# RustAudio/lewton

Measured on NVIDIA H100. Metric: Msamples/s IMDCT+window+OLA, 2048-pt long blocks, higher is better.
Workload: dtype f32

## Files before the change

lewton_b200/csrc/host_objects.cuh:

```cuda
#pragma once

struct DevBuf {
    void *p = nullptr;
    size_t cap = 0;
};

struct Staging {
    void *h = nullptr;
    size_t cap = 0;
    cudaEvent_t ev = nullptr;
    bool pending = false;
};

struct ArenaSet {
    DevBuf coeffs, dense, pcm, kinds, ys, vqoff, vqrec;
    cudaEvent_t done = nullptr;
};
constexpr int kHostSets = 2;

struct CachedTables {
    DevTables dt;
    std::vector<float> a, b, c, w;
    std::vector<uint32_t> br;
    std::vector<void *> allocs;
// ... 38 lines not shown
    lwb_ctx *ctx = nullptr;
    DevSetup host;
    DevSetup *d_setup = nullptr;
    std::vector<void *> allocs;
    uint8_t channels = 0, bs0 = 0, bs1 = 0;
    uint32_t n_modes = 0;
    uint32_t n_mappings = 0;
    std::vector<DevMapping> mappings;
    std::vector<uint8_t> floor_types;
    std::vector<DevFloor0> floor0;
    mutable bool streams_opened = false;
    bool floor0_described(uint32_t fi) const { return fi < floor0.size() && floor0[fi].order != 0; }
    unsigned out_channels() const { return host.n_out ? host.n_out : channels; }
};

struct RowCopy { const void *src; void *dst; uint64_t bytes; };
constexpr int kRowCopyThreads = 256;
struct ChainShape { unsigned warps; size_t smem; int n1max, wpc, np; };

struct Step {
    int kernel;
    const void *desc;
    size_t n;
    const float *pack;
};

struct StepArgs {
    void *pcm = nullptr;
    int out_format = LWB_OUT_F32_PLANAR;
    const float *w_short = nullptr;
    int ls = 0;
// ... 29 lines not shown
    lwb_batch_io io;
    bool captured = false;
    uint64_t gen = 0;
    FrontStages front;
    DevBuf pro, desc;
    StepArgs args;
    std::vector<Step> steps;
};

struct lwb_stream {
    lwb_ctx *ctx = nullptr;
    const lwb_setup *setup = nullptr;
    float *d_state = nullptr;
    bool has = false;
    uint32_t plen = 0;
    uint64_t busy_epoch = 0;
    uint64_t skip_left = 0;
    uint64_t limit_left = ~0ull;
};

static void capture(lwb_plan *plan, uint64_t gen, const FrontStages &front, const StepArgs &args, std::vector<Step> steps)
{
    plan->captured = true;
    plan->gen = gen;
    plan->front = front;
    for (size_t i = 0; i < plan->n_chains && front.n; i++)
        if (!plan->chains[i].stream->setup->floor0.empty()) plan->front.floor0 = true;
    plan->args = args;
    plan->steps = std::move(steps);
}


static inline void set_stream_state(lwb_stream *s, bool has, uint32_t plen)
{
    if (s->has != has || s->plen != plen) {
        s->has = has;
        s->plen = plen;
        s->ctx->state_gen++;
    }
}

static int fail(lwb_ctx *ctx, int code, const char *what, cudaError_t e = cudaSuccess)
{
    if (ctx) {
        ctx->err = what;
        if (e != cudaSuccess) {
            ctx->err += ": ";
            ctx->err += cudaGetErrorString(e);
        }
    }
    return code;
}
// ... 190 lines not shown
```

lewton_b200/csrc/kernel_long.cuh:

```cuda
#pragma once
#include <stdint.h>

#include "lwb_common.h"

#if defined(__CUDACC__)
#include <cuda_fp16.h>
#include <cuda_runtime.h>

#include <type_traits>
#define LWB_HD __host__ __device__ __forceinline__
#else
#define LWB_HD inline
#endif

namespace lwb {

constexpr int kLongBs = 11;
constexpr int kLongN = 2048;
constexpr int kLongN2 = 1024;

struct alignas(16) LongRun {
    const float *in;
    void *out;
    float *state;
    uint32_t in_stride;
    uint32_t n_packets;
    uint8_t has_prev;
    uint8_t write_state;
    uint8_t dummy;
    uint8_t first_short;
    uint8_t last_short;
    uint8_t pad[3];
    float *state_out;
};
static_assert(sizeof(LongRun) == 48, "LongRun is copied by TMA in 16-byte units");

struct V { float x, y; };

#if defined(__CUDA_ARCH__)
__device__ __forceinline__ V vadd(V a, V b) { return V{__fadd_rn(a.x, b.x), __fadd_rn(a.y, b.y)}; }
__device__ __forceinline__ V vsub(V a, V b) { return V{__fsub_rn(a.x, b.x), __fsub_rn(a.y, b.y)}; }
__device__ __forceinline__ V vmul(V a, V b) { return V{__fmul_rn(a.x, b.x), __fmul_rn(a.y, b.y)}; }
__device__ __forceinline__ V vadd_p(V a, V b) { return V{__fadd_rn(a.x, b.x), __fadd_rn(a.y, b.y)}; }
__device__ __forceinline__ V vsub_p(V a, V b) { return V{__fsub_rn(a.x, b.x), __fsub_rn(a.y, b.y)}; }
__device__ __forceinline__ V vnsub_p(V a, V b) { return V{__fsub_rn(-a.x, b.x), __fsub_rn(-a.y, b.y)}; }
#else
inline V vadd(V a, V b) { return V{a.x + b.x, a.y + b.y}; }
inline V vsub(V a, V b) { return V{a.x - b.x, a.y - b.y}; }
inline V vmul(V a, V b) { return V{a.x * b.x, a.y * b.y}; }
inline V vadd_p(V a, V b) { return vadd(a, b); }
// ... 348 lines not shown
__device__ __forceinline__ void mbar_wait(uint32_t bar, uint32_t parity)
{
    asm volatile(
        "{\n\t.reg .pred p;\n\t"
        "WAIT_%=:\n\t"
        "mbarrier.try_wait.parity.shared::cta.b64 p, [%0], %1, %2;\n\t"
        "@p bra DONE_%=;\n\t"
        "bra WAIT_%=;\n\t"
        "DONE_%=:\n\t}" ::"r"(bar), "r"(parity), "r"(200000u) : "memory");
}
__device__ __forceinline__ void tma_load_1d(uint32_t dst, const void *src, uint32_t bytes, uint32_t bar)
{
    asm volatile("cp.async.bulk.shared::cluster.global.mbarrier::complete_tx::bytes [%0], [%1], %2, [%3];"
                 ::"r"(dst), "l"(src), "r"(bytes), "r"(bar) : "memory");
}
__device__ __forceinline__ void fence_proxy_async()
{
    asm volatile("fence.proxy.async.shared::cta;" ::: "memory");
}
__device__ __forceinline__ void sts_eo(uint32_t addr, float e, float o)
{
    asm volatile("st.shared.f32 [%0], %1;\n\tst.shared.f32 [%0+2048], %2;" ::"r"(addr), "f"(e), "f"(o) : "memory");
}
__device__ __forceinline__ void lds_eo(uint32_t addr, float &e, float &o)
{
    asm volatile("ld.shared.f32 %0, [%2];\n\tld.shared.f32 %1, [%2+2048];" : "=f"(e), "=f"(o) : "r"(addr) : "memory");
}

}
#include "kernel_deal.cuh"
// ... 77 lines not shown
    case kSampleI16: return f(SampleType<int16_t>());
    case kSampleF16: return f(SampleType<__half>());
    default: return f(SampleType<float>());
    }
}

template <int FORMAT>
__device__ __forceinline__ void store_sample(void *pcm, uint64_t off, uint64_t stride, unsigned channels, unsigned ch,
                                             uint64_t i, float v)
{
    constexpr OutFormat F = out_format_of(FORMAT);
    using T = sample_t<F.kind>;
    static_cast<T *>(pcm)[off + (F.planar ? (uint64_t)ch * stride + i : i * channels + ch)] = d_sample(v, static_cast<T *>(nullptr));
}

template <int Wd, int TOP, bool FIRST, typename OutT>
__device__ __forceinline__ void out_block(const TwMix &tw, int hl, const V O[8], const V E[8], V pe[8], uint32_t flags,
                                          OutT *out, const float *s_state)
{
#pragma unroll
    for (int j = 0; j < 8; j++) {
        const int rw = Wd * rev3(j);
        const bool nat = (j & 1);
        const V b0 = tw(P_B0 + j), b1 = tw(P_B1 + j);
        const V wlo = tw(P_WLO + j), whi = tw(P_WHI + j);
        V plo = pe[j], phi = pe[j];
        bool emit = !(flags & 4u);
        if (FIRST) {
            emit = emit && (flags & 1u);
            if (flags & 1u) {
                const float *s_lo = s_state + hl, *s_hi = s_state + Wd - 1 - hl;
                const float ax = nat ? s_lo[rw] : s_hi[rw], ay = nat ? s_hi[rw] : s_lo[rw];
                const float bx = nat ? s_hi[TOP - rw] : s_lo[TOP - rw];
                const float by = nat ? s_lo[TOP - rw] : s_hi[TOP - rw];
                plo = V{ax, ay};
                phi = V{bx, by};
            }
        }
        V lo, hi, pev;
        step8_ola(b0, b1, wlo, whi, O[j], E[j], plo, phi, lo, hi, pev);
        pe[j] = pev;
        if (emit) {
            OutT *o_lo = out + hl, *o_hi = out + Wd - 1 - hl;
            if (nat) {
                st_pcm(o_lo + rw, lo.x); st_pcm(o_hi + rw, lo.y);
                st_pcm(o_hi + TOP - rw, hi.x); st_pcm(o_lo + TOP - rw, hi.y);
            } else {
                st_pcm(o_hi + rw, lo.x); st_pcm(o_lo + rw, lo.y);
                st_pcm(o_lo + TOP - rw, hi.x); st_pcm(o_hi + TOP - rw, hi.y);
            }
        }
    }
}

template <int NB, bool FIRST, typename OutT, typename RC>
__device__ __forceinline__ void out_stage(const TwMix &tw, int lane, const V O[NB][8], const V E[NB][8], V pe[NB][8],
                                          const RC cur[NB], OutT *out[NB], const float *s_state)
{
#pragma unroll
    for (int b = 0; b < NB; b++)
        out_block<64, kLongN2 - 64, FIRST>(tw, lane, O[b], E[b], pe[b], cur[b].flags, out[b], s_state + b * kLongN2);
}

__device__ __forceinline__ float lds_f32(uint32_t addr)
{
    float v;
    asm volatile("ld.shared.f32 %0, [%1];" : "=f"(v) : "r"(addr) : "memory");
    return v;
}

template <int NB, typename OutT, typename RC = RunCur, bool EXPORT = false, int LS = 0>
__device__ __forceinline__ void out_first_short(const TwMix &tw, int lane, const V O[NB][8], const V E[NB][8], V pe[NB][8],
                                                const RC cur[NB], OutT *out[NB], const float *s_state,
                                                const float *__restrict__ w, int ls_arg, uint32_t w_s = 0)
{
    const int ls = LS ? LS : ls_arg;
// ... 71 lines not shown
        }
    }
    __syncwarp();
#pragma unroll
    for (int b = 0; b < NB; b++) {
        const uint32_t c0 = stage_s + b * kLongTileBytes + lC0, c1 = stage_s + b * kLongTileBytes + lC1;
#pragma unroll
        for (int j = 0; j < 8; j++) {
            lds_eo(c0 ^ LWB_KC(j), E[b][j].x, O[b][j].x);
            lds_eo(c1 ^ LWB_KC(j), E[b][j].y, O[b][j].y);
        }
    }
    __syncwarp();
}

template <int Wd, int TOP>
__device__ __forceinline__ void store_right_half(float *state, int hl, const V pe[8])
{
    float *s_lo = state + hl, *s_hi = state + Wd - 1 - hl;
#pragma unroll
    for (int j = 0; j < 8; j++) {
        const int rw = Wd * rev3(j);
        const float vx = (j & 1) ? pe[j].x : pe[j].y, vy = (j & 1) ? pe[j].y : pe[j].x;
        s_lo[rw] = vx; s_hi[rw] = vy;
        s_hi[TOP - rw] = vx; s_lo[TOP - rw] = vy;
    }
}

template <int LS, typename OutT>
__device__ __forceinline__ void end_of_run(int lane, const V pe[8], uint32_t flags, uint32_t npk, OutT *out, float *state, int ls_arg)
{
    static_assert(LS % 64 == 0, "LS must be a multiple of 64");
    const int ls = LS ? LS : ls_arg;
    if (flags & 16u) {
        const bool emitted = (npk > 1 || (flags & 1u)) && !(flags & 4u);
        const bool keep = (flags & 6u) == 2u;
#pragma unroll
        for (int j = 0; j < 8; j++) {
            const int r64 = 64 * rev3(j);
#pragma unroll
            for (int h = 0; h < 2; h++) {
                const float v = ((j & 1) != 0) == (h == 0) ? pe[j].x : pe[j].y;
                const int m = r64 + (h ? 63 - lane : lane);
                if (LS ? (r64 < LS) : (m < ls)) {
                    if (emitted) st_pcm(out + m, v);
                } else if (keep && m < kLongN2 - ls) {
                    state[m - ls] = v;
                    state[kLongN2 - 1 - ls - m] = v;
                }
            }
        }
    } else if ((flags & 6u) == 2u) {
        store_right_half<64, kLongN2 - 64>(state, lane, pe);
    }
}

template <int Ring, size_t StageBytes, size_t Desc>
struct LongSmem {
    static constexpr size_t kTilesBytes = (size_t)kLongWarps * Ring * StageBytes;
    static constexpr size_t kStateBytes = (size_t)kLongWarps * StageBytes;
    static constexpr size_t kDescBytes = (size_t)kLongWarps * Desc * sizeof(LongRun);
    float *tiles, *s_state;
    V *s_pack;
    LongRun *s_desc;
    uint64_t *bars;
    unsigned char *rest;
    __device__ __forceinline__ LongSmem(unsigned char *smem_raw, int warp)
    {
// ... 69 lines not shown
    const uint32_t state_s = smem_u32(s_state), next_s = smem_u32(s_next);
    const uint32_t lA0 = laneA(lane, 0), lA1 = laneA(lane, 1);
    const uint32_t lB = laneB(lane);
    const uint32_t lC0 = laneC(lane, 0), lC1 = laneC(lane, 1);
    uint32_t phase_bits = 0;
    uint32_t slot_i = 0;

    uint32_t lc = 0;
    uint32_t nx_idx = 0;
    uint32_t nx_stage = 0;
    uint32_t nx_lc = 0, nx_npk = 0;
    uint32_t nx_state_issued = 0;
    uint32_t desc_parity = 0;
    RunCur cur[NB];
    uint32_t npk;

    auto issue_stage = [&](uint32_t stage, const auto *r, uint32_t pkt) {
        const uint32_t bar = bars_s + 8 * stage;
        mbar_expect_tx(bar, kLongStageBytes);
#pragma unroll
        for (int b = 0; b < NB; b++)
            tma_load_1d(tiles_s + stage * kLongStageBytes + b * kLongTileBytes,
                        r[b].in + (size_t)pkt * r[b].in_stride, kLongTileBytes, bar);
    };
    auto issue_state = [&](const float *const st[NB], const uint32_t has[NB]) {
        uint32_t bytes = 0;
#pragma unroll
        for (int b = 0; b < NB; b++) bytes += has[b] ? kLongTileBytes : 0;
        mbar_expect_tx(bar_state, bytes);
#pragma unroll
        for (int b = 0; b < NB; b++)
            if (has[b]) tma_load_1d(state_s + b * kLongTileBytes, st[b], kLongTileBytes, bar_state);
    };
    auto request_desc = [&]() {
        if (nx_idx < n_groups) {
            fence_proxy_async();
            mbar_expect_tx(bar_desc, NB * (uint32_t)sizeof(LongRun));
            tma_load_1d(next_s, runs + (size_t)nx_idx * NB, NB * (uint32_t)sizeof(LongRun), bar_desc);
            nx_stage = 1;
        } else {
            nx_stage = 3;
        }
    };
    auto land_desc = [&]() {
        mbar_wait(bar_desc, desc_parity);
        desc_parity ^= 1u;
        nx_stage = 2;
        nx_npk = s_next[0].n_packets;
        nx_lc = 0;
    };
    auto request_state = [&]() {
        const float *st[NB];
        uint32_t has[NB];
#pragma unroll
        for (int b = 0; b < NB; b++) { st[b] = s_next[b].state; has[b] = s_next[b].has_prev; }
        fence_proxy_async();
        issue_state(st, has);
        nx_state_issued = 1;
    };

    {
        uint32_t idx = 0;
        if (lane == 0) idx = atomicAdd(ticket, 1u);
        idx = __shfl_sync(0xffffffffu, idx, 0);
        if (idx >= n_groups) return;
#pragma unroll
        for (int b = 0; b < NB; b++) cur[b] = run_cur(runs[idx * NB + b]);
        npk = runs[idx * NB].n_packets;
        if (lane == 0) {
            fence_proxy_async();
            const float *st[NB];
            uint32_t has[NB];
#pragma unroll
            for (int b = 0; b < NB; b++) { st[b] = cur[b].state; has[b] = cur[b].flags & 1u; }
            issue_state(st, has);
            for (; lc < (uint32_t)kLongRing && lc < npk; lc++) issue_stage(lc, cur, lc);
            nx_idx = atomicAdd(ticket, 1u);
        }
    }

    for (;;) {
        V pe[NB][8];
#pragma unroll
        for (int b = 0; b < NB; b++)
#pragma unroll
            for (int j = 0; j < 8; j++) pe[b][j] = V{0.f, 0.f};
        OutT *out[NB];
#pragma unroll
        for (int b = 0; b < NB; b++) out[b] = static_cast<OutT *>(cur[b].out);

// ... 26 lines not shown
                            fence_proxy_async();
                            issue_stage(tgt, s_next, nx_lc);
                            nx_lc++;
                        }
                    }
                }
            }
            phase_c_fft<NB>(tw, O, E);
            if (p > 0) {
                out_stage<NB, false>(tw, lane, O, E, pe, cur, out, s_state);
            } else {
                mbar_wait(bar_state, (phase_bits >> 30) & 1u);
                phase_bits ^= 1u << 30;
                if (NB == 1 && (cur[0].flags & 8u))
                    out_first_short<NB, OutT>(tw, lane, O, E, pe, cur, out, s_state, w_short, ls);
                else
                    out_stage<NB, true>(tw, lane, O, E, pe, cur, out, s_state);
                __syncwarp();
            }
#pragma unroll
            for (int b = 0; b < NB; b++)
                if (p > 0 || (cur[b].flags & 1u)) out[b] += (p == 0 && (cur[b].flags & 8u)) ? kLongN2 - ls : kLongN2;
            if (lane == 0 && nx_stage == 2 && !nx_state_issued) request_state();
            slot_i = (slot_i + 1 == (uint32_t)kLongRing) ? 0 : slot_i + 1;
        }
#pragma unroll
        for (int b = 0; b < NB; b++) end_of_run<0>(lane, pe[b], cur[b].flags, npk, out[b], cur[b].state, ls);
        uint32_t st_ = 0, nlc = 0;
        if (lane == 0) {
            if (nx_stage == 0) request_desc();
            if (nx_stage == 1) land_desc();
            if (nx_stage == 2 && !nx_state_issued) request_state();
            st_ = nx_stage;
            nlc = nx_lc;
        }
        st_ = __shfl_sync(0xffffffffu, st_, 0);
        nlc = __shfl_sync(0xffffffffu, nlc, 0);
        if (st_ != 2) break;
        __syncwarp();
#pragma unroll
        for (int b = 0; b < NB; b++) cur[b] = run_cur(s_next[b]);
        npk = s_next[0].n_packets;
        __syncwarp();
        lc = nlc;
        nx_stage = 0; nx_lc = 0; nx_npk = 0; nx_state_issued = 0;
        if (lane == 0) {
            fence_proxy_async();
            for (uint32_t k = lc; k < (uint32_t)kLongRing && k < npk; k++) {
                issue_stage((slot_i + k) % kLongRing, cur, k);
                lc = k + 1;
            }
            nx_idx = atomicAdd(ticket, 1u);
        }
    }
}

// ... 138 lines not shown
```

lewton_b200/csrc/lwb_api.cu:

```cuda
#include <cuda_runtime.h>
#include <sched.h>
#include <sys/syscall.h>
#include <unistd.h>

#include <algorithm>
#include <cctype>
#include <cmath>
#include <cstdio>
#include <cstdlib>
#include <cstring>
#include <deque>
#include <new>
#include <string>
#include <vector>

#include "kernel_long.cuh"
#include "kernel_short.cuh"
#include "kernel_mid.cuh"
#include "kernels_generic.cuh"
#include "kernel_chain.cuh"
#include "kernel_prologue.cuh"
#include "kernel_floor0.cuh"
#include "lwb_common.h"
#include "pcm_copy_plan.h"
// ... 528 lines not shown
}

extern "C" void lwb_stream_destroy(lwb_stream *s)
{
    if (!s) return;
    cudaSetDevice(s->ctx->device);
    sync_all_streams(s->ctx);
    cudaFree(s->d_state);
    delete s;
}

extern "C" int lwb_stream_reset(lwb_stream *s)
{
    if (!s) return LWB_ERR_INVALID;
    set_stream_state(s, false, 0);
    return LWB_OK;
}
extern "C" int lwb_stream_set_window(lwb_stream *s, uint64_t skip, uint64_t limit)
{
    if (!s) return LWB_ERR_INVALID;
    s->skip_left = skip;
    s->limit_left = limit;
    s->ctx->windows_set = true;
    s->ctx->state_gen++;
    return LWB_OK;
}
extern "C" int lwb_stream_window(const lwb_stream *s, uint64_t *skip_left, uint64_t *limit_left)
{
    if (!s) return LWB_ERR_INVALID;
    if (skip_left) *skip_left = s->skip_left;
    if (limit_left) *limit_left = s->limit_left;
    return LWB_OK;
}
extern "C" int lwb_stream_is_empty(const lwb_stream *s) { return (!s || !s->has) ? 1 : 0; }
extern "C" uint32_t lwb_stream_state_len(const lwb_stream *s) { return (s && s->has) ? s->plen : 0; }

extern "C" int lwb_stream_clone(const lwb_stream *s, lwb_stream **out)
{
    if (!s || !out) return LWB_ERR_INVALID;
    int rc = lwb_stream_open(s->ctx, s->setup, out);
    if (rc) return rc;
    (*out)->has = s->has;
    (*out)->plen = s->plen;
    (*out)->skip_left = s->skip_left;
    (*out)->limit_left = s->limit_left;
    lwb_ctx *ctx = s->ctx;
    CU(ctx, cudaMemcpyAsync((*out)->d_state, s->d_state,
                            s->setup->channels * state_stride(s->setup) * sizeof(float),
                            cudaMemcpyDeviceToDevice, ctx->stream));
    return LWB_OK;
}

extern "C" int lwb_stream_export_state(lwb_stream *s, float *out)
{
    if (!s || !out) return LWB_ERR_INVALID;
    if (!s->has) return LWB_OK;
    lwb_ctx *ctx = s->ctx;
    CU(ctx, cudaSetDevice(ctx->device));
    CU(ctx, cudaMemcpy2DAsync(out, s->plen * sizeof(float), s->d_state, state_stride(s->setup) * sizeof(float),
                              s->plen * sizeof(float), s->setup->channels, cudaMemcpyDeviceToHost, ctx->stream));
    CU(ctx, cudaStreamSynchronize(ctx->stream));
    return LWB_OK;
}

extern "C" int lwb_stream_import_state(lwb_stream *s, const float *data, uint32_t len)
{
    if (!s || (!data && len)) return LWB_ERR_INVALID;
    if (len > state_stride(s->setup)) return LWB_ERR_BUFFER;
    lwb_ctx *ctx = s->ctx;
    CU(ctx, cudaSetDevice(ctx->device));
    if (len) {
        CU(ctx, cudaMemcpy2DAsync(s->d_state, state_stride(s->setup) * sizeof(float), data, len * sizeof(float),
                                  len * sizeof(float), s->setup->channels, cudaMemcpyHostToDevice, ctx->stream));
        CU(ctx, cudaStreamSynchronize(ctx->stream));
    }
    s->ctx->state_gen++;
    s->has = true;
    s->plen = len;
    return LWB_OK;
}

extern "C" int lwb_decoded_sample_count(const lwb_setup *su, uint8_t mode, int prev_flag, int next_flag,
                                        uint32_t *n_samples)
{
    if (!su || !n_samples) return LWB_ERR_INVALID;
    Geom g;
    int rc = geometry(su, mode, prev_flag, next_flag, &g);
    if (rc) return rc;
    *n_samples = g.rs - g.ls;
    return LWB_OK;
}

#include "path_generic.cuh"
// ... 122 lines not shown
static int queue_batch(lwb_ctx *ctx, lwb_chain *chains, size_t n_chains, const lwb_batch_io *io, lwb_plan *prepared, bool pinned_only)
{
    if (!ctx || (!chains && n_chains) || !io) return LWB_ERR_INVALID;
    BatchWalk bw;
    int rc = walk_batch(ctx, chains, n_chains, io, pinned_only, &bw);
    if (rc || n_chains == 0) return rc;
    CU(ctx, cudaSetDevice(ctx->device));
    if ((rc = place_clipped_chains(ctx, chains, n_chains, io, &bw))) return rc;
    const lwb_chain *decode = bw.clip.empty() ? chains : bw.clip.data();
    if (prepared) prepared->captured = false;
    size_t first = first_batch_path();
    for (size_t i = 0; i < n_chains && first < kChainPath; i++)
        if (chains[i].stream->setup->host.n_out) first = kChainPath;
    for (size_t k = first; k < std::size(kBatchPaths); k++) {
        bool handled = false;
        if ((rc = kBatchPaths[k](ctx, decode, n_chains, io, bw, &handled, prepared))) return rc;
        if (!handled) continue;
        if (prepared && !bw.clip.empty()) prepared->captured = false;
        for (size_t i = 0; i < n_chains; i++) set_chain_result(&chains[i], bw.walks[i]);
        commit_stream_states(chains, bw.walks);
        return LWB_OK;
    }
    return fail(ctx, LWB_ERR_INVALID, "internal: no batch path took the batch");
}

static int decode_chains_impl(lwb_ctx *ctx, lwb_chain *chains, size_t n_chains, const lwb_batch_io *io, lwb_plan *prepared,
                              uint64_t *ticket = nullptr)
{
    if (!ctx) return LWB_ERR_INVALID;
    const uint64_t issued = ctx->tickets_issued;
    int rc = queue_batch(ctx, chains, n_chains, io, prepared, ticket != nullptr);
    if (rc) return rc;
    if (!ticket) return ctx->tickets_issued != issued ? retire_tickets(ctx, ctx->tickets_issued, true) : LWB_OK;
    if (ctx->tickets_issued == issued) {
        CU(ctx, cudaSetDevice(ctx->device));
// ... 71 lines not shown
{
    size_t rows = 0;
    for (size_t i = 0; i < n; i++)
        if (slot_len(slots[i], load)) rows += slots[i].stream->setup->channels;
    if (!rows) return LWB_OK;
    Staging *st;
    int rc;
    if ((rc = acquire_staging(ctx, rows * sizeof(RowCopy), &st)) || (rc = ensure(ctx, ctx->state_rows, rows * sizeof(RowCopy)))) return rc;
    RowCopy *h = (RowCopy *)st->h;
    size_t k = 0;
    for (size_t i = 0; i < n; i++) {
        const lwb_stream *s = slots[i].stream;
        const uint32_t len = slot_len(slots[i], load);
        for (unsigned c = 0; len && c < s->setup->channels; c++) {
            float *row = s->d_state + (size_t)c * state_stride(s->setup), *b = dev + (slots[i].offset - base) + (uint64_t)c * len;
            h[k++] = load ? RowCopy{b, row, len * sizeof(float)} : RowCopy{row, b, len * sizeof(float)};
        }
    }
    if ((rc = upload_staging(ctx, st, h, ctx->state_rows.p, rows * sizeof(RowCopy), ctx->stream))) return rc;
    return run_steps(ctx, StepArgs(), std::vector<Step>(1, Step{LWB_KERNEL_ROW_COPY, ctx->state_rows.p, rows, nullptr}));
}

static int move_states(lwb_ctx *ctx, bool load, lwb_state_slot *slots_w, const lwb_state_slot *slots, size_t n, int memory, float *buf,
                       uint64_t *ticket)
{
    uint64_t lo, hi;
    int rc = check_state_slots(ctx, slots, n, memory, buf, ticket, load, &lo, &hi);
    if (rc) return rc;
    CU(ctx, cudaSetDevice(ctx->device));
    ArenaSet *set = nullptr;
    if (memory == LWB_MEM_DEVICE || hi <= lo) {
// ... 26 lines not shown
            }
        }
        if (rc) {
            cudaEventRecord(set->done, ctx->stream);
            cudaGetLastError();
            return rc;
        }
    }
    if ((rc = issue_ticket(ctx, set))) return rc;
    *ticket = ctx->tickets_issued;
    for (size_t i = 0; i < n; i++) {
        lwb_stream *s = slots[i].stream;
        if (load) {
            s->has = slots[i].has != 0;
            s->plen = slots[i].len;
        } else {
            slots_w[i].len = slot_len(slots[i], false);
            slots_w[i].has = s->has ? 1 : 0;
        }
    }
    if (load) ctx->state_gen++;
    return LWB_OK;
}

extern "C" int lwb_streams_save(lwb_ctx *ctx, lwb_state_slot *slots, size_t n, int memory, float *buf, uint64_t *ticket)
{
    return move_states(ctx, false, slots, slots, n, memory, buf, ticket);
}

extern "C" int lwb_streams_load(lwb_ctx *ctx, const lwb_state_slot *slots, size_t n, int memory, const float *buf, uint64_t *ticket)
// ... 189 lines not shown
```

lewton_b200/csrc/path_chain.cuh:

```cuda
#pragma once

static size_t chain_smem(unsigned maxc, int n1max, int np, bool vq = false)
{
    return (size_t)maxc * ((size_t)np * n1max + n1max / 2) * 4 + 8 * (LWB_MAX_POSTS + 1) * 2 * 2 + 64 +
           (vq ? (size_t)maxc * (n1max / 2) * 4 : 0);
}
static int chain_np(unsigned maxc, int n1max, int wpc, bool residue)
{
    if (residue || wpc != 1) return 1;
    int np = 4;
    while (np > 1 && chain_smem(maxc, n1max, np) > 64 * 1024) np >>= 1;
    return np;
}
static ChainShape chain_shape(unsigned maxc, int n1max, bool residue, bool vq = false)
{
    int wpc = std::max(1, std::min(8, n1max / 1024));
    while (wpc > 1 && (unsigned)wpc * maxc > 32) wpc >>= 1;
    const int np = chain_np(maxc, n1max, wpc, residue);
    return ChainShape{maxc * wpc, chain_smem(maxc, n1max, np, vq), n1max, wpc, np};
}

template <int Q>
__device__ __forceinline__ void row_copy_shifted(const uint4 *__restrict__ a, uint4 *__restrict__ d, uint64_t nv, unsigned r)
{
    for (uint64_t v = threadIdx.x; v < nv; v += blockDim.x) {
        const uint4 A = a[v], B = a[v + 1];
        const uint32_t w[8] = {A.x, A.y, A.z, A.w, B.x, B.y, B.z, B.w};
        d[v] = make_uint4(__funnelshift_r(w[Q], w[Q + 1], r), __funnelshift_r(w[Q + 1], w[Q + 2], r), __funnelshift_r(w[Q + 2], w[Q + 3], r),
                          __funnelshift_r(w[Q + 3], w[Q + 4], r));
    }
}

__global__ void __launch_bounds__(kRowCopyThreads) k_row_copy(const RowCopy *__restrict__ rc)
{
    const RowCopy c = rc[blockIdx.x];
    const char *src = static_cast<const char *>(c.src);
    char *dst = static_cast<char *>(c.dst);
    const uint64_t head = min(c.bytes, (uint64_t)((16 - (reinterpret_cast<uintptr_t>(dst) & 15)) & 15));
    const uint64_t nv = (c.bytes - head) >> 4;
    for (uint64_t i = 2 * threadIdx.x; i < head; i += 2 * blockDim.x)
        *reinterpret_cast<uint16_t *>(dst + i) = *reinterpret_cast<const uint16_t *>(src + i);
    for (uint64_t i = head + nv * 16 + 2 * threadIdx.x; i < c.bytes; i += 2 * blockDim.x)
        *reinterpret_cast<uint16_t *>(dst + i) = *reinterpret_cast<const uint16_t *>(src + i);
    uint4 *d = reinterpret_cast<uint4 *>(dst + head);
    const char *s = src + head;
    const unsigned sh = reinterpret_cast<uintptr_t>(s) & 15, r = (sh & 3) * 8;
    const uint4 *a = reinterpret_cast<const uint4 *>(s - sh);
    switch (sh >> 2) {
    case 0:
        if (!sh) {
// ... 123 lines not shown
```

lewton_b200/csrc/path_generic.cuh:

```cuda
#pragma once

struct ChainWalk {
    uint32_t done = 0;
    int status = LWB_OK;
    uint64_t n_samples = 0;
    uint64_t skip = 0;
    uint64_t written = 0;
    bool end_has = false;
    uint32_t end_plen = 0;
    bool clear_after = false;
    uint64_t coeff_end = 0;
    uint32_t full_n = 0;
    bool long_only = true;
    bool clipped() const { return skip || written != n_samples; }
};

template <typename F>
static ChainWalk walk_chain(const lwb_chain *c, F &&on_packet)
{
    const lwb_setup *su = c->stream->setup;
    ChainWalk w;
    bool has = c->stream->has;
    uint32_t plen = c->stream->plen;
    uint64_t coeff = c->coeff_offset, pos = 0;
// ... 398 lines not shown
    for (size_t i = i0; i < i1; i++) {
        const lwb_chain *c = &chains[i];
        pcm_chain_spans(planar, c->stream->setup->out_channels(), c->out_offset, c->out_stride, walks[i].written, ctx->pcm_spans);
    }
    plan_pcm_copies(ctx->pcm_spans, (uint64_t)INT32_MAX / esz, ctx->pcm_copies);
    for (const PcmCopy &cp : ctx->pcm_copies) {
        char *dst = (char *)io->pcm + cp.off * esz;
        const char *src = (const char *)stage + (cp.off - obase) * esz;
        if (cp.height == 1) CU(ctx, cudaMemcpyAsync(dst, src, cp.width * esz, cudaMemcpyDeviceToHost, st));
        else CU(ctx, cudaMemcpy2DAsync(dst, cp.pitch * esz, src, cp.pitch * esz, cp.width * esz, cp.height, cudaMemcpyDeviceToHost, st));
    }
    return LWB_OK;
}

static int run_steps(lwb_ctx *ctx, const StepArgs &a, const std::vector<Step> &steps);

struct BatchArenas {
    const float *coeffs = nullptr, *dense = nullptr;
    char *pcm = nullptr;
    FloorViews fl;
    lwb_ctx *ctx = nullptr;
    const lwb_batch_io *io = nullptr;
    ArenaSet *set = nullptr;
    bool host = false;
    unsigned C = 0;
    uint64_t c_lo = 0, o_lo = 0;
    cudaStream_t up = nullptr, down = nullptr;

    int open(lwb_ctx *ctx_, const lwb_batch_io *io_, const BatchExtent &ext, unsigned C_, bool copy_streams)
    {
// ... 412 lines not shown
```

lewton_b200/csrc/path_long.cuh:

```cuda
#pragma once

struct LongItem {
    const lwb_chain *c;
    uint32_t P;
    bool has_prev;
};

static void long_runs_of(const LongItem &it, size_t cuts, const float *coeffs, char *pcm, size_t esz, LongRun *&w)
{
    for (unsigned ch = 0; ch < it.c->stream->setup->channels; ch++, w += cuts)
        channel_run(it.c, ch, kLongN2, coeffs + it.c->coeff_offset, pcm, esz, it.P, it.has_prev, it.has_prev ? kLongN2 : 0, cuts, w);
}

static bool batch_is_uniform_long(const lwb_chain *chains, size_t n_chains, const lwb_batch_io *io, const BatchWalk &bw)
{
    if (!fused_layout(chains, n_chains, io)) return false;
    const float *pack = nullptr;
    for (size_t i = 0; i < n_chains; i++) {
        const lwb_chain *c = &chains[i];
        const lwb_stream *s = c->stream;
        const lwb_setup *su = s->setup;
        if (su->bs1 != kLongBs || !su->host.tab[1].pack) return false;
        if (pack && pack != su->host.tab[1].pack) return false;
        pack = su->host.tab[1].pack;
        if (s->has && s->plen != (uint32_t)kLongN2) return false;
        if (bw.walks[i].done != c->n_packets || !bw.walks[i].long_only) return false;
    }
    return true;
}

struct LongRuns {
    struct Chunk { size_t r0, nr; };
    std::vector<Chunk> chunks;
    Staging *st = nullptr;
    LongRun *h = nullptr, *d = nullptr;
    size_t n = 0;
    int par = 0;
    bool own = false;
};

static int long_build_runs(lwb_ctx *ctx, const lwb_chain *chains, size_t n_chains, size_t n_chunks, const float *coeffs, char *pcm,
                           size_t esz, DevBuf *own, LongRuns *lr)
{
    std::vector<LongItem> items;
    items.reserve(n_chains);
    size_t chan_chains = 0;
    for (size_t i = 0; i < n_chains; i++) {
        const lwb_chain *c = &chains[i];
        items.push_back(LongItem{c, c->n_packets, c->stream->has});
        if (c->n_packets) chan_chains += c->stream->setup->channels;
    }
    const size_t warp_slots = (size_t)ctx->sm_count * kLongWarps * kLongNB;
    size_t target_runs = warp_slots * 4;
    if (const char *e = getenv("LWB_LONG_TARGET_RUNS")) target_runs = (size_t)atol(e);
    const size_t min_run = 8;
    int rc;
    std::vector<size_t> cuts(items.size(), 1);
// ... 18 lines not shown
    lr->h = h_runs;
    std::vector<LongRun> tmp;
    std::vector<uint32_t> order;
    for (size_t k = 0; k < n_chunks; k++) {
        const size_t i0 = items.size() * k / n_chunks, i1 = items.size() * (k + 1) / n_chunks;
        LongRun *w0 = w;
        size_t chunk_runs = 0;
        for (size_t i = i0; i < i1; i++)
            if (items[i].P) chunk_runs += cuts[i] * items[i].c->stream->setup->channels;
        LongRun *gen = w;
        if (kLongNB > 1) {
            tmp.resize(chunk_runs);
            gen = tmp.data();
        }
        for (size_t i = i0; i < i1; i++)
            if (items[i].P) long_runs_of(items[i], cuts[i], coeffs, pcm, esz, gen);
        if (kLongNB == 1) {
            w = gen;
        } else {
            bool sorted = true;
            for (size_t i = 1; i < tmp.size() && sorted; i++) sorted = tmp[i].n_packets == tmp[0].n_packets;
            order.resize(tmp.size());
            for (uint32_t i = 0; i < order.size(); i++) order[i] = i;
            if (!sorted)
                std::stable_sort(order.begin(), order.end(),
                                 [&](uint32_t a, uint32_t b) { return tmp[a].n_packets < tmp[b].n_packets; });
            size_t i = 0;
            while (i < order.size()) {
                size_t j = i;
                while (j < order.size() && tmp[order[j]].n_packets == tmp[order[i]].n_packets) j++;
                for (size_t q = i; q < j; q++) *w++ = tmp[order[q]];
// ... 60 lines not shown
    StepArgs args;
    args.pcm = ar.pcm;
    args.out_format = io->out_format;
    std::vector<Step> steps;
    LongRuns lr;
    uint64_t gen = 0;
    size_t pk0 = 0;
    for (size_t k = 0; k < n_chunks; k++) {
        const size_t i0 = n_chains * k / n_chunks, i1 = n_chains * (k + 1) / n_chunks;
        const BatchExtent ke = chunk_extent(io, chains, bw, i0, i1);
        if (ke.empty()) continue;
        size_t npk = 0;
        for (size_t i = i0; i < i1; i++) npk += chains[i].n_packets;
        if ((rc = ar.upload(k, ke)) || (residue && (rc = front_stages_launch(ctx, ar, fs, pk0, npk)))) return rc;
        if (!lr.d) {
            if ((rc = long_build_runs(ctx, chains, n_chains, n_chunks, in, ar.pcm, out_format_of(io->out_format).esz, cap ? &plan->desc : nullptr, &lr)) ||
                (rc = long_upload_runs(ctx, lr, host ? ctx->copy_in : ctx->copy_out)))
                return rc;
            gen = ctx->state_gen;
        }
        steps.assign(1, Step{LWB_KERNEL_LONG, lr.d + lr.chunks[k].r0, lr.chunks[k].nr / kLongNB, pack});
        if ((rc = run_steps(ctx, args, steps)) || (rc = ar.download(k, bw, i0, i1, ke))) return rc;
        pk0 += npk;
    }
    CU(ctx, cudaEventRecord(ctx->ev_kdone[lr.par], ctx->stream));
    if (cap) capture(plan, gen, fs, args, std::move(steps));
    return ar.finish();
}
```

Before: 323,500.

## Store only half of long-block overlap state and mirror it lazily

The long-block kernel keeps only the non-redundant half of the symmetric overlap-add state when running under a captured plan. It writes half the state rows with an L2 evict_last hint and reads them back with half-size TMA loads. Other batch paths, state export and slot save rebuild the full mirrored rows through a mirror mode in the row-copy kernel. This halves state traffic per run, but adds a stream flag, generation bumps and an extra mirroring launch whenever a non-long path reads the state.

New measurement: 332,000 (median of 6 runs). +2.6%, better.

```diff
diff --git a/lewton_b200/csrc/host_objects.cuh b/lewton_b200/csrc/host_objects.cuh
--- a/lewton_b200/csrc/host_objects.cuh
+++ b/lewton_b200/csrc/host_objects.cuh
@@ -76,7 +76,7 @@
     unsigned out_channels() const { return host.n_out ? host.n_out : channels; }
 };
 
-struct RowCopy { const void *src; void *dst; uint64_t bytes; };
+struct RowCopy { const void *src; void *dst; uint64_t bytes; bool mirror = false; };
 constexpr int kRowCopyThreads = 256;
 struct ChainShape { unsigned warps; size_t smem; int n1max, wpc, np; };
 
@@ -136,6 +136,7 @@
     float *d_state = nullptr;
     bool has = false;
     uint32_t plen = 0;
+    bool half = false;
     uint64_t busy_epoch = 0;
     uint64_t skip_left = 0;
     uint64_t limit_left = ~0ull;
@@ -158,6 +159,14 @@
     if (s->has != has || s->plen != plen) {
         s->has = has;
         s->plen = plen;
+        s->ctx->state_gen++;
+    }
+}
+
+static inline void set_stream_half(lwb_stream *s, bool half)
+{
+    if (s->half != half) {
+        s->half = half;
         s->ctx->state_gen++;
     }
 }
diff --git a/lewton_b200/csrc/kernel_long.cuh b/lewton_b200/csrc/kernel_long.cuh
--- a/lewton_b200/csrc/kernel_long.cuh
+++ b/lewton_b200/csrc/kernel_long.cuh
@@ -30,10 +30,12 @@
     uint8_t dummy;
     uint8_t first_short;
     uint8_t last_short;
-    uint8_t pad[3];
+    uint8_t half;
+    uint8_t pad[2];
     float *state_out;
 };
 static_assert(sizeof(LongRun) == 48, "LongRun is copied by TMA in 16-byte units");
+constexpr uint8_t kLongHalfIn = 1, kLongHalfOut = 2;
 
 struct V { float x, y; };
 
@@ -412,6 +414,16 @@
     asm volatile("cp.async.bulk.shared::cluster.global.mbarrier::complete_tx::bytes [%0], [%1], %2, [%3];"
                  ::"r"(dst), "l"(src), "r"(bytes), "r"(bar) : "memory");
 }
+__device__ __forceinline__ uint64_t l2_evict_last_policy()
+{
+    uint64_t p;
+    asm volatile("createpolicy.fractional.L2::evict_last.b64 %0, 1.0;" : "=l"(p));
+    return p;
+}
+__device__ __forceinline__ void st_f32_policy(float *p, float v, uint64_t pol)
+{
+    asm volatile("st.global.L2::cache_hint.f32 [%0], %1, %2;" ::"l"(p), "f"(v), "l"(pol) : "memory");
+}
 __device__ __forceinline__ void fence_proxy_async()
 {
     asm volatile("fence.proxy.async.shared::cta;" ::: "memory");
@@ -519,7 +531,7 @@
     static_cast<T *>(pcm)[off + (F.planar ? (uint64_t)ch * stride + i : i * channels + ch)] = d_sample(v, static_cast<T *>(nullptr));
 }
 
-template <int Wd, int TOP, bool FIRST, typename OutT>
+template <int Wd, int TOP, bool FIRST, typename OutT, bool HALF = false>
 __device__ __forceinline__ void out_block(const TwMix &tw, int hl, const V O[8], const V E[8], V pe[8], uint32_t flags,
                                           OutT *out, const float *s_state)
 {
@@ -536,10 +548,14 @@
             if (flags & 1u) {
                 const float *s_lo = s_state + hl, *s_hi = s_state + Wd - 1 - hl;
                 const float ax = nat ? s_lo[rw] : s_hi[rw], ay = nat ? s_hi[rw] : s_lo[rw];
-                const float bx = nat ? s_hi[TOP - rw] : s_lo[TOP - rw];
-                const float by = nat ? s_lo[TOP - rw] : s_hi[TOP - rw];
                 plo = V{ax, ay};
-                phi = V{bx, by};
+                if (HALF) {
+                    phi = plo;
+                } else {
+                    const float bx = nat ? s_hi[TOP - rw] : s_lo[TOP - rw];
+                    const float by = nat ? s_lo[TOP - rw] : s_hi[TOP - rw];
+                    phi = V{bx, by};
+                }
             }
         }
         V lo, hi, pev;
@@ -558,13 +574,13 @@
     }
 }
 
-template <int NB, bool FIRST, typename OutT, typename RC>
+template <int NB, bool FIRST, bool HALF = false, typename OutT, typename RC>
 __device__ __forceinline__ void out_stage(const TwMix &tw, int lane, const V O[NB][8], const V E[NB][8], V pe[NB][8],
                                           const RC cur[NB], OutT *out[NB], const float *s_state)
 {
 #pragma unroll
     for (int b = 0; b < NB; b++)
-        out_block<64, kLongN2 - 64, FIRST>(tw, lane, O[b], E[b], pe[b], cur[b].flags, out[b], s_state + b * kLongN2);
+        out_block<64, kLongN2 - 64, FIRST, OutT, HALF>(tw, lane, O[b], E[b], pe[b], cur[b].flags, out[b], s_state + b * kLongN2);
 }
 
 __device__ __forceinline__ float lds_f32(uint32_t addr)
@@ -666,7 +682,7 @@
     __syncwarp();
 }
 
-template <int Wd, int TOP>
+template <int Wd, int TOP, bool HALF = false>
 __device__ __forceinline__ void store_right_half(float *state, int hl, const V pe[8])
 {
     float *s_lo = state + hl, *s_hi = state + Wd - 1 - hl;
@@ -674,12 +690,17 @@
     for (int j = 0; j < 8; j++) {
         const int rw = Wd * rev3(j);
         const float vx = (j & 1) ? pe[j].x : pe[j].y, vy = (j & 1) ? pe[j].y : pe[j].x;
-        s_lo[rw] = vx; s_hi[rw] = vy;
-        s_hi[TOP - rw] = vx; s_lo[TOP - rw] = vy;
-    }
-}
-
-template <int LS, typename OutT>
+        if (HALF) {
+            const uint64_t pol = l2_evict_last_policy();
+            st_f32_policy(s_lo + rw, vx, pol); st_f32_policy(s_hi + rw, vy, pol);
+        } else {
+            s_lo[rw] = vx; s_hi[rw] = vy;
+            s_hi[TOP - rw] = vx; s_lo[TOP - rw] = vy;
+        }
+    }
+}
+
+template <int LS, bool HALF = false, typename OutT>
 __device__ __forceinline__ void end_of_run(int lane, const V pe[8], uint32_t flags, uint32_t npk, OutT *out, float *state, int ls_arg)
 {
     static_assert(LS % 64 == 0, "LS must be a multiple of 64");
@@ -703,7 +724,8 @@
             }
         }
     } else if ((flags & 6u) == 2u) {
-        store_right_half<64, kLongN2 - 64>(state, lane, pe);
+        if (HALF && (flags & 128u)) store_right_half<64, kLongN2 - 64, true>(state, lane, pe);
+        else store_right_half<64, kLongN2 - 64>(state, lane, pe);
     }
 }
 
@@ -803,6 +825,11 @@
     uint32_t desc_parity = 0;
     RunCur cur[NB];
     uint32_t npk;
+    auto run_cur_l = [](const LongRun &r) {
+        RunCur c = run_cur(r);
+        if (NB == 1) c.flags |= (uint32_t)(r.half & (kLongHalfIn | kLongHalfOut)) << 6;
+        return c;
+    };
 
     auto issue_stage = [&](uint32_t stage, const auto *r, uint32_t pkt) {
         const uint32_t bar = bars_s + 8 * stage;
@@ -812,14 +839,17 @@
             tma_load_1d(tiles_s + stage * kLongStageBytes + b * kLongTileBytes,
                         r[b].in + (size_t)pkt * r[b].in_stride, kLongTileBytes, bar);
     };
-    auto issue_state = [&](const float *const st[NB], const uint32_t has[NB]) {
-        uint32_t bytes = 0;
-#pragma unroll
-        for (int b = 0; b < NB; b++) bytes += has[b] ? kLongTileBytes : 0;
+    auto issue_state = [&](const float *const st[NB], const uint32_t fl[NB]) {
+        uint32_t bytes = 0, sz[NB];
+#pragma unroll
+        for (int b = 0; b < NB; b++) {
+            sz[b] = !(fl[b] & 1u) ? 0u : (fl[b] & 64u) ? kLongTileBytes / 2 : kLongTileBytes;
+            bytes += sz[b];
+        }
         mbar_expect_tx(bar_state, bytes);
 #pragma unroll
         for (int b = 0; b < NB; b++)
-            if (has[b]) tma_load_1d(state_s + b * kLongTileBytes, st[b], kLongTileBytes, bar_state);
+            if (sz[b]) tma_load_1d(state_s + b * kLongTileBytes, st[b], sz[b], bar_state);
     };
     auto request_desc = [&]() {
         if (nx_idx < n_groups) {
@@ -840,11 +870,11 @@
     };
     auto request_state = [&]() {
         const float *st[NB];
-        uint32_t has[NB];
-#pragma unroll
-        for (int b = 0; b < NB; b++) { st[b] = s_next[b].state; has[b] = s_next[b].has_prev; }
+        uint32_t fl[NB];
+#pragma unroll
+        for (int b = 0; b < NB; b++) { st[b] = s_next[b].state; fl[b] = run_cur_l(s_next[b]).flags; }
         fence_proxy_async();
-        issue_state(st, has);
+        issue_state(st, fl);
         nx_state_issued = 1;
     };
 
@@ -854,15 +884,15 @@
         idx = __shfl_sync(0xffffffffu, idx, 0);
         if (idx >= n_groups) return;
 #pragma unroll
-        for (int b = 0; b < NB; b++) cur[b] = run_cur(runs[idx * NB + b]);
+        for (int b = 0; b < NB; b++) cur[b] = run_cur_l(runs[idx * NB + b]);
         npk = runs[idx * NB].n_packets;
         if (lane == 0) {
             fence_proxy_async();
             const float *st[NB];
-            uint32_t has[NB];
-#pragma unroll
-            for (int b = 0; b < NB; b++) { st[b] = cur[b].state; has[b] = cur[b].flags & 1u; }
-            issue_state(st, has);
+            uint32_t fl[NB];
+#pragma unroll
+            for (int b = 0; b < NB; b++) { st[b] = cur[b].state; fl[b] = cur[b].flags; }
+            issue_state(st, fl);
             for (; lc < (uint32_t)kLongRing && lc < npk; lc++) issue_stage(lc, cur, lc);
             nx_idx = atomicAdd(ticket, 1u);
         }
@@ -919,6 +949,8 @@
                 phase_bits ^= 1u << 30;
                 if (NB == 1 && (cur[0].flags & 8u))
                     out_first_short<NB, OutT>(tw, lane, O, E, pe, cur, out, s_state, w_short, ls);
+                else if (NB == 1 && (cur[0].flags & 64u))
+                    out_stage<NB, true, true>(tw, lane, O, E, pe, cur, out, s_state);
                 else
                     out_stage<NB, true>(tw, lane, O, E, pe, cur, out, s_state);
                 __syncwarp();
@@ -930,7 +962,7 @@
             slot_i = (slot_i + 1 == (uint32_t)kLongRing) ? 0 : slot_i + 1;
         }
 #pragma unroll
-        for (int b = 0; b < NB; b++) end_of_run<0>(lane, pe[b], cur[b].flags, npk, out[b], cur[b].state, ls);
+        for (int b = 0; b < NB; b++) end_of_run<0, true>(lane, pe[b], cur[b].flags, npk, out[b], cur[b].state, ls);
         uint32_t st_ = 0, nlc = 0;
         if (lane == 0) {
             if (nx_stage == 0) request_desc();
@@ -944,7 +976,7 @@
         if (st_ != 2) break;
         __syncwarp();
 #pragma unroll
-        for (int b = 0; b < NB; b++) cur[b] = run_cur(s_next[b]);
+        for (int b = 0; b < NB; b++) cur[b] = run_cur_l(s_next[b]);
         npk = s_next[0].n_packets;
         __syncwarp();
         lc = nlc;
diff --git a/lewton_b200/csrc/lwb_api.cu b/lewton_b200/csrc/lwb_api.cu
--- a/lewton_b200/csrc/lwb_api.cu
+++ b/lewton_b200/csrc/lwb_api.cu
@@ -566,6 +566,7 @@
 {
     if (!s) return LWB_ERR_INVALID;
     set_stream_state(s, false, 0);
+    set_stream_half(s, false);
     return LWB_OK;
 }
 extern "C" int lwb_stream_set_window(lwb_stream *s, uint64_t skip, uint64_t limit)
@@ -594,6 +595,7 @@
     if (rc) return rc;
     (*out)->has = s->has;
     (*out)->plen = s->plen;
+    (*out)->half = s->half;
     (*out)->skip_left = s->skip_left;
     (*out)->limit_left = s->limit_left;
     lwb_ctx *ctx = s->ctx;
@@ -612,6 +614,8 @@
     CU(ctx, cudaMemcpy2DAsync(out, s->plen * sizeof(float), s->d_state, state_stride(s->setup) * sizeof(float),
                               s->plen * sizeof(float), s->setup->channels, cudaMemcpyDeviceToHost, ctx->stream));
     CU(ctx, cudaStreamSynchronize(ctx->stream));
+    for (unsigned c = 0; s->half && c < s->setup->channels; c++)
+        for (uint32_t m = 0; m < s->plen / 2; m++) out[(size_t)c * s->plen + s->plen - 1 - m] = out[(size_t)c * s->plen + m];
     return LWB_OK;
 }
 
@@ -629,6 +633,7 @@
     s->ctx->state_gen++;
     s->has = true;
     s->plen = len;
+    s->half = false;
     return LWB_OK;
 }
 
@@ -781,11 +786,17 @@
         if (chains[i].stream->setup->host.n_out) first = kChainPath;
     for (size_t k = first; k < std::size(kBatchPaths); k++) {
         bool handled = false;
+        if (kBatchPaths[k] != try_long &&
+            (rc = materialise_halves(ctx, n_chains, [&](size_t i) { return chains[i].stream; }, [&](size_t i) { return bw.walks[i].done > 0; })))
+            return rc;
         if ((rc = kBatchPaths[k](ctx, decode, n_chains, io, bw, &handled, prepared))) return rc;
         if (!handled) continue;
         if (prepared && !bw.clip.empty()) prepared->captured = false;
         for (size_t i = 0; i < n_chains; i++) set_chain_result(&chains[i], bw.walks[i]);
         commit_stream_states(chains, bw.walks);
+        if (kBatchPaths[k] == try_long)
+            for (size_t i = 0; i < n_chains; i++)
+                if (bw.walks[i].done) set_stream_half(chains[i].stream, prepared != nullptr);
         return LWB_OK;
     }
     return fail(ctx, LWB_ERR_INVALID, "internal: no batch path took the batch");
@@ -887,7 +898,7 @@
         const uint32_t len = slot_len(slots[i], load);
         for (unsigned c = 0; len && c < s->setup->channels; c++) {
             float *row = s->d_state + (size_t)c * state_stride(s->setup), *b = dev + (slots[i].offset - base) + (uint64_t)c * len;
-            h[k++] = load ? RowCopy{b, row, len * sizeof(float)} : RowCopy{row, b, len * sizeof(float)};
+            h[k++] = load ? RowCopy{b, row, len * sizeof(float)} : RowCopy{row, b, len * sizeof(float), s->half};
         }
     }
     if ((rc = upload_staging(ctx, st, h, ctx->state_rows.p, rows * sizeof(RowCopy), ctx->stream))) return rc;
@@ -944,6 +955,7 @@
         if (load) {
             s->has = slots[i].has != 0;
             s->plen = slots[i].len;
+            s->half = false;
         } else {
             slots_w[i].len = slot_len(slots[i], false);
             slots_w[i].has = s->has ? 1 : 0;
diff --git a/lewton_b200/csrc/path_chain.cuh b/lewton_b200/csrc/path_chain.cuh
--- a/lewton_b200/csrc/path_chain.cuh
+++ b/lewton_b200/csrc/path_chain.cuh
@@ -34,6 +34,17 @@
 __global__ void __launch_bounds__(kRowCopyThreads) k_row_copy(const RowCopy *__restrict__ rc)
 {
     const RowCopy c = rc[blockIdx.x];
+    if (c.mirror) {
+        const float *s = static_cast<const float *>(c.src);
+        float *d = static_cast<float *>(c.dst);
+        const uint64_t n = c.bytes / 4;
+        for (uint64_t m = threadIdx.x; m < n / 2; m += blockDim.x) {
+            const float v = s[m];
+            d[m] = v;
+            d[n - 1 - m] = v;
+        }
+        return;
+    }
     const char *src = static_cast<const char *>(c.src);
     char *dst = static_cast<char *>(c.dst);
     const uint64_t head = min(c.bytes, (uint64_t)((16 - (reinterpret_cast<uintptr_t>(dst) & 15)) & 15));
diff --git a/lewton_b200/csrc/path_generic.cuh b/lewton_b200/csrc/path_generic.cuh
--- a/lewton_b200/csrc/path_generic.cuh
+++ b/lewton_b200/csrc/path_generic.cuh
@@ -436,6 +436,33 @@
 }
 
 static int run_steps(lwb_ctx *ctx, const StepArgs &a, const std::vector<Step> &steps);
+
+template <typename StreamAt, typename Reads>
+static int materialise_halves(lwb_ctx *ctx, size_t n, StreamAt &&streams, Reads &&read)
+{
+    size_t rows = 0;
+    for (size_t i = 0; i < n; i++)
+        if (streams(i)->half && read(i)) rows += streams(i)->setup->channels;
+    if (!rows) return LWB_OK;
+    Staging *st;
+    int rc;
+    if ((rc = acquire_staging(ctx, rows * sizeof(RowCopy), &st)) || (rc = ensure(ctx, ctx->state_rows, rows * sizeof(RowCopy)))) return rc;
+    RowCopy *h = (RowCopy *)st->h;
+    size_t k = 0;
+    for (size_t i = 0; i < n; i++) {
+        const lwb_stream *s = streams(i);
+        for (unsigned c = 0; s->half && read(i) && c < s->setup->channels; c++) {
+            float *row = s->d_state + (size_t)c * state_stride(s->setup);
+            h[k++] = RowCopy{row, row, state_stride(s->setup) * sizeof(float), true};
+        }
+    }
+    if ((rc = upload_staging(ctx, st, h, ctx->state_rows.p, rows * sizeof(RowCopy), ctx->stream)) ||
+        (rc = run_steps(ctx, StepArgs(), std::vector<Step>(1, Step{LWB_KERNEL_ROW_COPY, ctx->state_rows.p, rows, nullptr}))))
+        return rc;
+    for (size_t i = 0; i < n; i++)
+        if (read(i)) set_stream_half(streams(i), false);
+    return LWB_OK;
+}
 
 struct BatchArenas {
     const float *coeffs = nullptr, *dense = nullptr;
diff --git a/lewton_b200/csrc/path_long.cuh b/lewton_b200/csrc/path_long.cuh
--- a/lewton_b200/csrc/path_long.cuh
+++ b/lewton_b200/csrc/path_long.cuh
@@ -6,10 +6,13 @@
     bool has_prev;
 };
 
-static void long_runs_of(const LongItem &it, size_t cuts, const float *coeffs, char *pcm, size_t esz, LongRun *&w)
+static void long_runs_of(const LongItem &it, size_t cuts, const float *coeffs, char *pcm, size_t esz, bool halves, LongRun *&w)
 {
-    for (unsigned ch = 0; ch < it.c->stream->setup->channels; ch++, w += cuts)
+    const uint8_t half = (it.c->stream->half ? kLongHalfIn : 0) | (halves ? kLongHalfOut : 0);
+    for (unsigned ch = 0; ch < it.c->stream->setup->channels; ch++, w += cuts) {
         channel_run(it.c, ch, kLongN2, coeffs + it.c->coeff_offset, pcm, esz, it.P, it.has_prev, it.has_prev ? kLongN2 : 0, cuts, w);
+        for (size_t k = 0; k < cuts; k++) w[k].half = half;
+    }
 }
 
 static bool batch_is_uniform_long(const lwb_chain *chains, size_t n_chains, const lwb_batch_io *io, const BatchWalk &bw)
@@ -40,7 +43,7 @@
 };
 
 static int long_build_runs(lwb_ctx *ctx, const lwb_chain *chains, size_t n_chains, size_t n_chunks, const float *coeffs, char *pcm,
-                           size_t esz, DevBuf *own, LongRuns *lr)
+                           size_t esz, DevBuf *own, bool halves, LongRuns *lr)
 {
     std::vector<LongItem> items;
     items.reserve(n_chains);
@@ -89,7 +92,7 @@
             gen = tmp.data();
         }
         for (size_t i = i0; i < i1; i++)
-            if (items[i].P) long_runs_of(items[i], cuts[i], coeffs, pcm, esz, gen);
+            if (items[i].P) long_runs_of(items[i], cuts[i], coeffs, pcm, esz, halves, gen);
         if (kLongNB == 1) {
             w = gen;
         } else {
@@ -180,7 +183,7 @@
         for (size_t i = i0; i < i1; i++) npk += chains[i].n_packets;
         if ((rc = ar.upload(k, ke)) || (residue && (rc = front_stages_launch(ctx, ar, fs, pk0, npk)))) return rc;
         if (!lr.d) {
-            if ((rc = long_build_runs(ctx, chains, n_chains, n_chunks, in, ar.pcm, out_format_of(io->out_format).esz, cap ? &plan->desc : nullptr, &lr)) ||
+            if ((rc = long_build_runs(ctx, chains, n_chains, n_chunks, in, ar.pcm, out_format_of(io->out_format).esz, cap ? &plan->desc : nullptr, plan != nullptr, &lr)) ||
                 (rc = long_upload_runs(ctx, lr, host ? ctx->copy_in : ctx->copy_out)))
                 return rc;
             gen = ctx->state_gen;
diff --git a/profiles/long_state_bench.py b/profiles/long_state_bench.py
--- /dev/null
+++ b/profiles/long_state_bench.py
@@ -0,0 +1,91 @@
+import argparse
+import json
+import os
+import subprocess
+import sys
+
+import numpy as np
+
+sys.path.insert(0, os.path.dirname(os.path.dirname(os.path.abspath(__file__))))
+
+import lewton_b200 as L
+from lewton_b200 import _cabi as cabi
+
+N2 = 1024
+FLUSH_BYTES = 128 << 20
+
+
+def gpu_info():
+    import torch
+    name = torch.cuda.get_device_name(0)
+    try:
+        q = subprocess.run(["nvidia-smi", "--query-gpu=power.limit,clocks.sm,clocks.max.sm", "--format=csv,noheader", "-i", "0"],
+                           capture_output=True, text=True, timeout=30).stdout.strip()
+    except (OSError, subprocess.SubprocessError):
+        q = "unknown"
+    return name, q
+
+
+def main():
+    import torch
+    ap = argparse.ArgumentParser()
+    ap.add_argument("--streams", type=int, default=4096)
+    ap.add_argument("--steps", type=int, default=20, help="timed steps per round and case")
+    ap.add_argument("--rounds", type=int, default=5)
+    args = ap.parse_args()
+    S, Ch = args.streams, 2
+    ctx = L.Context(0)
+    su = L.Setup(ctx, Ch, 8, 11, [L.FloorTypeOne(1, [0, 128])], [L.Mapping(Ch)], [L.ModeInfo(False), L.ModeInfo(True)])
+    stream = torch.cuda.ExternalStream(ctx.cuda_stream, device=torch.device("cuda", 0))
+    flush = torch.empty(FLUSH_BYTES // 4, dtype=torch.float32, device="cuda")
+
+    cases = {}
+    for name, P, fmt, esz, flushed in (("f32_16", 16, cabi.OUT_F32_PLANAR, 4, False), ("f32_64", 64, cabi.OUT_F32_PLANAR, 4, False),
+                                       ("f16_16", 16, cabi.OUT_F16_PLANAR, 2, False), ("f32_16_flushed", 16, cabi.OUT_F32_PLANAR, 4, True)):
+        gen = torch.Generator(device="cuda").manual_seed(1234)
+        spec = torch.randn((S, P, Ch, N2), generator=gen, device="cuda", dtype=torch.float32) * 1e-2
+        pcm = torch.empty((S, Ch, P * N2), device="cuda", dtype=torch.float16 if esz == 2 else torch.float32)
+        pwrs = [L.PreviousWindowRight(su) for _ in range(S)]
+        chains = [L.ChainSpec(pwrs[s], np.ones(P, np.uint8), coeff_offset=s * P * Ch * N2, out_offset=s * Ch * P * N2, out_stride=P * N2)
+                  for s in range(S)]
+        batch = L.Batch(ctx, chains, cabi.ENTRY_SPECTRUM, cabi.MEM_DEVICE, spec.data_ptr(), pcm.data_ptr(), fmt)
+        for _ in range(5):
+            batch.run()
+        samples = S * P * Ch * N2
+        state_half, state_full = S * Ch * 2 * (N2 // 2) * 4, S * Ch * 2 * N2 * 4
+        cases[name] = dict(P=P, flushed=flushed, batch=batch, keep=(spec, pcm, pwrs), samples=samples,
+                           io_bytes=samples * 4 + samples * esz, state_half=state_half, state_full=state_full, ms=[])
+    ctx.synchronize()
+    torch.cuda.synchronize()
+
+    ev = [(torch.cuda.Event(enable_timing=True), torch.cuda.Event(enable_timing=True)) for _ in range(args.steps)]
+    for _ in range(args.rounds):
+        for c in cases.values():
+            c["batch"].run()
+            for e0, e1 in ev:
+                if c["flushed"]:
+                    with torch.cuda.stream(stream):
+                        flush.fill_(1.0)
+                e0.record(stream)
+                c["batch"].run()
+                e1.record(stream)
+            ctx.synchronize()
+            torch.cuda.synchronize()
+            c["ms"].append(sum(e0.elapsed_time(e1) for e0, e1 in ev) / args.steps)
+
+    name, q = gpu_info()
+    out = {"gpu": name, "power_limit, sm_clock, max_sm_clock": q, "streams": S, "steps": args.steps, "rounds": args.rounds, "cases": {}}
+    for k, c in cases.items():
+        ms = float(np.median(c["ms"]))
+        tb = lambda b: b / (ms * 1e-3) / 1e12
+        out["cases"][k] = {"packets": c["P"], "ms_per_step": ms, "ms_min": min(c["ms"]), "ms_max": max(c["ms"]),
+                           "Msamples_per_s": c["samples"] / (ms * 1e-3) / 1e6,
+                           "MB_per_step_halves": (c["io_bytes"] + c["state_half"]) / 1e6, "TBps_halves": tb(c["io_bytes"] + c["state_half"]),
+                           "MB_per_step_full_rows": (c["io_bytes"] + c["state_full"]) / 1e6, "TBps_full_rows": tb(c["io_bytes"] + c["state_full"])}
+    f, u = out["cases"]["f32_16_flushed"]["ms_per_step"], out["cases"]["f32_16"]["ms_per_step"]
+    out["l2_residency_share_ms"] = f - u
+    print(json.dumps(out))
+
+
+if __name__ == "__main__":
+    main()
```
